# zeahmed/NeuralASR

Hardware: AMD Instinct MI355X
Metric: audio-frames/sec (fwd+bwd+CTC+Adam) at batch 16 per GPU (higher is better)
Workload: dtype f32

## Files before the change

neuralasr_amd/build.py:

```python
import os
import subprocess
import sys
from concurrent.futures import ThreadPoolExecutor

HERE = os.path.dirname(os.path.abspath(__file__))
CSRC = os.path.join(HERE, 'csrc')
LIB = os.path.join(HERE, 'libnasr.so')
KT_LIB = os.path.join(HERE, 'libnasr_kt.so')
KT_SRC = os.path.join(HERE, '..', 'tests', 'kernel_harness', 'harness.hip')
KT_OBJS = ['gemm.o', 'gemm_tph.o', 'optim.o']
SOURCES = ['gemm.hip', 'gemm_tph.hip', 'lstm.hip', 'lstm_persist.hip', 'lstm_wide.hip', 'ctc.hip', 'dense.hip', 'optim.hip', 'nasr_layout.hip',
           'nasr_rec.hip', 'nasr_batch.hip', 'nasr_pass.hip', 'nasr_api.hip', 'nasr_comm.hip', 'beam.cpp',
           'wavenet.hip', 'nasr_wavenet.hip', 'las.hip', 'las_beam.hip', 'nasr_las.hip', 'mfcc.hip', 'resample.hip']
HEADERS = [os.path.join(CSRC, 'kernels.h'), os.path.join(CSRC, 'lstm_device.h'), os.path.join(CSRC, 'nasr_ctx.h'), os.path.join(CSRC, 'wavenet.h'), os.path.join(CSRC, 'las.h'), os.path.join(CSRC, 'las_beam.h'), os.path.join(CSRC, 'resample.h'),
           os.path.join(HERE, '..', 'include', 'nasr.h')]
FLAGS = ['--offload-arch=gfx950', '-O3', '-std=c++17', '-fPIC', '-Wall', '-Wno-unused-function']


def _hipcc():
    for c in (os.environ.get('HIPCC'), '/opt/rocm/bin/hipcc', 'hipcc'):
        if c and (os.path.isabs(c) and os.path.exists(c) or not os.path.isabs(c)):
            return c
    return 'hipcc'


def _stale(target, deps):
    if not os.path.exists(target):
        return True
    t = os.path.getmtime(target)
    return any(os.path.getmtime(d) > t for d in deps if os.path.exists(d))


def build(force=False, verbose=False):
    hipcc = _hipcc()
    bdir = os.path.join(HERE, 'build')
    os.makedirs(bdir, exist_ok=True)
    jobs = []
    objs = []
    for s in SOURCES:
        src = os.path.join(CSRC, s)
        obj = os.path.join(bdir, os.path.splitext(s)[0] + '.o')
        objs.append(obj)
        if force or _stale(obj, [src] + HEADERS):
            jobs.append([hipcc] + FLAGS + ['-c', src, '-o', obj])

    def run(cmd):
        if verbose:
            print(' '.join(cmd), flush=True)
        r = subprocess.run(cmd, capture_output=True, text=True)
        if r.returncode != 0:
            raise RuntimeError('hipcc failed:\n' + ' '.join(cmd) + '\n' + r.stdout + r.stderr)
        if verbose and r.stderr.strip():
            print(r.stderr)

    kt_obj = os.path.join(bdir, 'kt_harness.o')
    if force or _stale(kt_obj, [KT_SRC] + HEADERS):
        jobs.append([hipcc] + FLAGS + ['-c', KT_SRC, '-o', kt_obj])

    with ThreadPoolExecutor(max_workers=min(4, max(1, len(jobs)))) as ex:
        list(ex.map(run, jobs))
    if force or jobs or _stale(LIB, objs):
        run([hipcc, '--offload-arch=gfx950', '-shared', '-fPIC', '-o', LIB] + objs + ['-lpthread'])
    kt_objs = [kt_obj] + [os.path.join(bdir, o) for o in KT_OBJS]
    if force or jobs or _stale(KT_LIB, kt_objs):
# ... 7 lines not shown
```

neuralasr_amd/csrc/kernels.h:

```cpp
#pragma once
#include <hip/hip_runtime.h>
#include <stdint.h>

namespace nasr {

const char* test_hook(const char* name);

struct GemmDesc {
  const float* A;
  const float* B;
  float* C;
  int M, N, K;
  int lda, ldb, ldc;
  bool a_col;
  bool b_col;
  const int* a_map;
  int a_shift;
  int a_rows;
  const int* c_map;
  const float* bias;
  int split_k;
  float* slabs;
};
void launch_gemm(const GemmDesc& g, hipStream_t st);
int gemm_pick_split(int M, int N, int K);

int tp_split2_parts(int rows);
int gemm_tp_tile_rows(int M);
size_t tph_bytes(int rows, int K);
size_t tph_scale_ws_floats(int rows, int K);
void launch_tph_scales(const float* src, int rows, int K, int ld, float* row_scale, float* row_inv, float* col_scale,
                       float* col_inv, float* ws, hipStream_t st);
constexpr int TPH_MAX_JOBS = 16;
struct TphScaleJob { const float* src; int rows, K, ld; float *row_scale, *row_inv, *col_scale, *col_inv; };
size_t tph_scale_batch_ws_floats(const TphScaleJob* jobs, int n);
void launch_tph_scales_batch(const TphScaleJob* jobs, int n, float* ws, hipStream_t st);
void launch_tph_scales_from_parts(const float* rowpart, int nrp, int rows, float* row_scale, float* row_inv, const float* colpart,
                                  int ncp, int K, float* col_scale, float* col_inv, hipStream_t st);
void launch_fill(float* p, float v, int n, hipStream_t st);
void launch_tph_split2(const float* src, unsigned char* tpN, unsigned char* tpT, int rows, int K, int ld,
                       const float* row_scale, float rs, const float* col_scale, float cs, float* colpart, hipStream_t st,
                       const int* rowmap = nullptr, const int* rowmap2 = nullptr, int col2 = 0);
void launch_gather_rows(float* dst, const float* src, const int* map, int n, float fill, hipStream_t st);
struct GemmTPHDesc {
  const unsigned char* A;
  const unsigned char* B;
  float* C;
  int M, N, K;
  int nkbA, nkbB;
  int ldc;
  int a_kshift;
  const float* bias;
  const float* a_inv;
  const float* b_inv;
  int split_k;
  float* slabs;
  int tile_rows;
  int nbatch;
  size_t a_bstride, b_bstride;
  int64_t c_bstride, ainv_bstride, binv_bstride;
  int a_kshift1;
  bool side;
  const int* c_map;
};
hipError_t gemm_tph_prepare();
int gemm_tph_pick_split(int M, int N, int K, int nbatch = 1);
void launch_gemm_tph(const GemmTPHDesc& g, hipStream_t st);

struct LstmDims {
  int T, B, Bp, H, Hp, D;
};
void launch_pack_feats(const float* feats_bm, float* X0, int B, int Bp, int T, int F, int Fp, hipStream_t st);
void launch_expand_context(const float* centre, const float* pad, const int* seq_len, float* X0, int B, int Bp, int T,
                           int ctx, int ncep, int Fp, hipStream_t st);
void launch_expand_context_masked(const float* centre, const float* pad, const int* seq_len, const int* masks, int nm,
                                  int static_width, float* X0, int B, int Bp, int T, int ctx, int ncep, int Fp,
                                  hipStream_t st);
void launch_repack_u(const float* U, float* Uf, float* Ub, int Hp, hipStream_t st);
// ... 102 lines not shown
```

neuralasr_amd/csrc/nasr_ctx.h:

```cpp
#pragma once
#include <hip/hip_runtime.h>

#include <dlfcn.h>
#include <sched.h>
#include <unistd.h>

#include <chrono>

#include <algorithm>
#include <cmath>
#include <cstdio>
#include <cstdlib>
#include <cstring>
#include <functional>
#include <map>
#include <memory>
#include <mutex>
#include <string>
#include <vector>

#include "../../include/nasr.h"
#include "kernels.h"
#include "resample.h"

// ... 117 lines not shown
  bool has_labels = false, centre = false;
  int64_t frames = 0;
  size_t o_seq = 0, o_lablen = 0, o_labels = 0, o_cstart = 0, o_cpos = 0, o_rowmap = 0;
  size_t o_vrow = 0, o_vprev = 0, o_vnext = 0;
  int Rv = 0, Rvp = 0;
  bool cmp = false;
  size_t nmeta = 0, nfeat = 0;
  size_t o_aug = 0;
  int aug_nm = 0, aug_sw = 0;
  bool masked = false;
  int32_t* meta_d() const { return dmeta.as<int32_t>(); }
};

enum class RecKind { Step = 0, Persist = 1, Wide = 2 };

enum class Family { Lstm, WaveNet, Las, Featurizer };

struct WnState;
struct WnStateDelete { void operator()(WnState* w) const; };
struct FzState;
struct FzStateDelete { void operator()(FzState* f) const; };
struct LasState;
struct LasStateDelete { void operator()(LasState* s) const; };

}

using namespace nasr;
using namespace nasr_impl;

struct nasr_ctx {

  nasr_model_cfg cfg;
  Family family = Family::Lstm;
  std::unique_ptr<WnState, WnStateDelete> wn;
  std::unique_ptr<FzState, FzStateDelete> fz;
  std::unique_ptr<LasState, LasStateDelete> las;
  int device = 0;
  Stream st;
  DevPtr<unsigned char> WfTP;
  DevPtr<unsigned char> WbTP;
  std::vector<size_t> off_wftp, off_wbtp;
  RecKind rec_kind = RecKind::Step;
  RecKind rec_use = RecKind::Step;
  bool rec_wanted = false;
  bool rec_inflight = false;
  bool rec_refused = false;
  int64_t rearm_after = 0, rearm_wait = 0, clean_steps = 0;
  int persist_aborts = 0, persist_rearms = 0;
  Pinned<unsigned> perr;
  DevPtr<float> Ucs, Ucinv;
  bool rec_f16 = false;
  DevPtr<float> Upf, Upb;
  size_t imf = 0, imb = 0;
  DevPtr<float> xchf;
  DevPtr<float> xchb;
  DevPtr<PersistCtl> pctl;
  DevPtr<unsigned char> Uw;
  DevPtr<unsigned char> Uwb;
  DevPtr<float> Urs, Urinv;
  DevPtr<float> wsrow;
  DevPtr<void> whx;
  DevPtr<float> wpart;
  DevPtr<void> wpx;
  DevPtr<WideCtl> wctl;
  void* comm = nullptr;
  void* comm2 = nullptr;
  Stream comm_st2;
  int comm_rank = 0, comm_n = 1;
  Stream comm_st;
  Event ev_comm;
  DevPtr<float> comm_scratch;

  int F, Fp, H, Hp, N4, D, L, C, Cp, Pin, Pinp;
  std::vector<int> Ip;
  std::vector<int64_t> off_wx, off_bias;
  std::vector<int64_t> off_u;
  int64_t off_w = 0, off_b = 0, np_int = 0;
  std::vector<TensorInfo> tensors;
  int64_t np_tf = 0;
  std::vector<int32_t> tf2int;

  int npre = 0, ndense = 0;
  bool has_post = false;
  int F0 = 0;
  std::vector<int> dWid, dWp, dIn, dIp;
  std::vector<int64_t> off_dw, off_db;
  std::vector<size_t> off_dftp, off_dbtp;
  DevPtr<unsigned char> DfTP, DbTP;
  std::vector<DevBuf> Ybuf, dYbuf;
  DevBuf DTP;
  uint32_t drop_seed = 4567u, drop_counter = 0;

  DevPtr<float> P, M, V, Uf, Ub;
  float* G = nullptr;
  struct SV {
    DevBuf s, inv;
    bool ensure(size_t n) { bool g = false; return s.ensure(n * 4, &g) && inv.ensure(n * 4, &g); }
    float* sp() const { return s.as<float>(); }
    float* ip() const { return inv.as<float>(); }
  };
  SV sc15;
  size_t sc15_n = 0;
  SV sc_x0r, sc_x0c;
  std::vector<SV> sc_yr, sc_yc;
  SV sc_gr, sc_gc;
  std::vector<SV> sc_wr, sc_wc;
  std::vector<SV> sc_dr, sc_dc;
  DevBuf scws;
  int gttp_layer = -1;
// ... 248 lines not shown
```

neuralasr_amd/csrc/nasr_pass.hip:

```cpp
#include "nasr_ctx.h"

using namespace nasr;
using namespace nasr_impl;

namespace nasr_impl {

int run_steps(nasr_ctx* h, int l, bool bwd, int s0, int s1, hipStream_t st, int* launches) {
  if (h->rec_use != RecKind::Step && s0 == 0 && s1 == h->T) return rec_launch(h, l, bwd, st, launches);
  *launches += s1 - s0;
  const LstmDims dm{h->T, h->B, h->Bp, h->H, h->Hp, h->D};
  const size_t sU = (size_t)l * h->D * h->Hp * h->N4;
  const size_t hs = (size_t)h->D * h->Bp * h->Hp;
  const size_t ps = (size_t)h->D * lstm_bwd_partials(h->Hp) * h->Bp * h->Hp;
  float* hst = h->hstate.as<float>();
  float* par = h->partial.as<float>();
  float* dcs = h->dcstate.as<float>();
  auto body = [&]() {
    if (!bwd) {
      if (s0 == 0) (void)hipMemsetAsync(hst, 0, hs * 4, st);
      for (int s = s0; s < s1; ++s)
        launch_lstm_fwd_step(dm, s, h->Uf + sU, hst + (s & 1) * hs, hst + ((s + 1) & 1) * hs,
                             h->gates[l].as<float>(), h->cbuf[l].as<float>(), h->outb[l].as<float>(),
                             h->seq_p, h->cfg.forget_bias, st);
    } else {
// ... 112 lines not shown
  pl_gemm(g, as.rinv, h->sc_dc[i].ip(), h->st);
  launch_dense_act(h->Ybuf[i].as<float>(), R, h->Bp, h->B, h->dWid[i], Wp, h->cfg.relu_clip, h->cfg.dropout[i],
                   h->drop_seed, h->drop_counter, i, h->st);
  pl_scales(h, h->Ybuf[i].as<float>(), R, Wp, Wp, &h->sc_yr[i], &h->sc_yc[i], h->st);
  HIPCHK(h, hipGetLastError());
  return NASR_OK;
}

int dense_backward(nasr_ctx* h, int i, const float* X, float* dX) {
  const int R = h->T * h->Bp, Ip = h->dIp[i], Wp = h->dWp[i];
  const int nkb = (R + 15) / 16;
  float* dZ = h->dYbuf[i].as<float>();
  launch_dense_act_bwd(dZ, h->Ybuf[i].as<float>(), (int64_t)R * Wp, h->cfg.relu_clip, h->cfg.dropout[i], h->st);
  const ActScale as = dense_in_scale(h, i);
  pl_scales(h, dZ, R, Wp, Wp, dX ? &h->sc_gr : nullptr, &h->sc_gc, h->st);
  pl_split(dZ, dX ? h->GTP.as<unsigned char>() : nullptr, h->GTTP.as<unsigned char>(), R, Wp, Wp, h->sc_gr.sp(),
           h->sc_gc.sp(), h->csws.as<float>(), h->st);
  pl_split(X, nullptr, h->DTP.as<unsigned char>(), R, Ip, Ip, nullptr, as.cs, nullptr, h->st);
  {
    GemmTPHDesc g{};
    g.A = h->DTP.as<unsigned char>(); g.B = h->GTTP.as<unsigned char>(); g.C = h->G + h->off_dw[i];
    g.M = Ip; g.N = Wp; g.K = R; g.nkbA = nkb; g.nkbB = nkb; g.ldc = Wp;
    g.split_k = gemm_tph_pick_split(g.M, g.N, g.K);
    g.slabs = ensure_slabs(h, g.split_k, g.M, g.N);
    if (g.split_k > 1 && !g.slabs) return h->fail(NASR_ERR_HIP, "slab workspace allocation failed");
    pl_gemm(g, as.cinv, h->sc_gc.ip(), h->st);
  }
  launch_colsum_parts(h->csws.as<float>(), tp_split2_parts(R), Wp, h->G + h->off_db[i], h->st);
  if (dX) {
    GemmTPHDesc g{};
    g.A = h->GTP.as<unsigned char>(); g.B = h->DbTP + h->off_dbtp[i]; g.C = dX;
    g.M = R; g.N = Ip; g.K = Wp; g.nkbA = (Wp + 15) / 16; g.nkbB = g.nkbA; g.ldc = Ip;
    g.split_k = gemm_tph_pick_split(g.M, g.N, g.K);
    g.slabs = ensure_slabs(h, g.split_k, g.M, g.N);
    if (g.split_k > 1 && !g.slabs) g.split_k = 1;
    pl_gemm(g, h->sc_gr.ip(), h->sc_dr[i].ip(), h->st);
  }
  HIPCHK(h, hipGetLastError());
  return NASR_OK;
}

int forward(nasr_ctx* h) {
  if (!h->resident) return h->fail(NASR_ERR_STATE, "no resident batch: call nasr_upload_batch first");
  switch (h->family) {
    case Family::WaveNet: return wn_forward(h, false);
    case Family::Las: return h->fail(NASR_ERR_STATE, "a LAS handle has no CTC logits: use nasr_las_forward");
    default: break;
  }
  const int Bp = h->Bp, T = h->T, D = h->D, Hp = h->Hp;
  const int R = T * Bp;
  h->n_fwd_launch = 0;
  std::fill(h->ott_valid.begin(), h->ott_valid.end(), 0);
  HIPCHK(h, hipMemsetAsync(h->Gbase, 0, GRAD_HEAD * 4, h->st));
  if (h->rec_use == RecKind::Persist) {
    HIPCHK(h, hipMemsetAsync(h->pctl + 1, 0, (size_t)h->L * sizeof(PersistCtl), h->st));
    HIPCHK(h, hipMemsetAsync(h->xchf, 0, (size_t)h->L * persist_hx_bytes(h->Hp), h->st));
  }
  for (int i = 0; i < h->npre; ++i) {
    PhaseScope ps(h, PH_XPROJ);
    int rc = dense_forward(h, i, i == 0 ? h->X0.as<float>() : h->Ybuf[i - 1].as<float>());
    if (rc) return rc;
  }
  for (int l = 0; l < h->L; ++l) {
    {
      PhaseScope ps(h, PH_XPROJ);
      gemm_xproj(h, l, R, h->st);
      HIPCHK(h, hipGetLastError());
    }
    PhaseScope ps(h, PH_RECF);
    int rc = run_steps(h, l, false, 0, T, h->st, &h->n_fwd_launch);
    if (rc) return rc;
  }
  if (h->has_post) {
    PhaseScope ps(h, PH_XPROJ);
    int rc = dense_forward(h, h->npre, h->outb[h->L - 1].as<float>());
    if (rc) return rc;
  }
  if (h->ndense) h->drop_counter += 1;
  {
    PhaseScope ps(h, PH_PROJCTC);
    const bool sr = h->cfg.merge == NASR_MERGE_STACK_RESHAPE && D == 2;
    GemmDesc g{};
    g.A = h->has_post ? h->Ybuf[h->npre].as<float>() : h->outb[h->L - 1].as<float>();
    g.B = h->P + h->off_w;
    g.C = h->logits.as<float>();
    g.M = h->Tp * Bp; g.N = h->Cp; g.K = h->Pinp;
    g.lda = sr ? Hp : h->Pinp; g.ldb = h->Cp; g.ldc = h->Cp;
    g.a_map = sr ? h->rowmap_p : nullptr;
    g.a_rows = sr ? 2 * R : R;
    g.bias = h->P + h->off_b;
    g.split_k = gemm_pick_split(g.M, g.N, g.K);
    if (int rc = gemm_f32(h, g)) return rc;
  }
  h->have_fwd = true;
  return NASR_OK;
}

CtcDims ctc_dims(nasr_ctx* h) {
  CtcDims d;
  d.Tp = h->Tp; d.B = h->B; d.Bp = h->Bp; d.C = h->C; d.Cp = h->Cp; d.Lmax = std::max(h->Lmax, 1);
  d.KS = h->KS; d.Tws = h->T + 8;
  d.lprobs = h->ctcprobs.as<float>(); d.goff = h->ctckexp.as<double>();
  return d;
}

int ctc_forward(nasr_ctx* h) {
  PhaseScope ps(h, PH_PROJCTC);
  const CtcDims d = ctc_dims(h);
  launch_ctc_logz(d, h->logits.as<float>(), h->seq_p, h->logz.as<float>(), h->st);
  launch_ctc_alpha_beta(d, h->logits.as<float>(), h->logz.as<float>(), h->labels_p, h->lablen_p,
                        h->seq_p, h->alpha.as<float>(), h->beta.as<float>(), h->aoff.as<double>(),
                        h->boff.as<double>(), h->nll.as<float>(), h->logp.as<double>(), h->st);
  launch_mean(h->nll.as<float>(), h->B, h->loss.as<float>(), h->st);
  if (h->step_decode) {
    if (h->step_greedy)
      launch_greedy(d, h->logits.as<float>(), h->seq_p, h->amax.as<int>(), h->ids.as<int>(), h->lens.as<int>(), h->st);
    h->have_decoded = h->step_greedy;
    h->res_cur ^= 1;
    nasr_ctx::StepRes& r = h->res[h->res_cur];
    const size_t ids_bytes = 8 + (size_t)h->Bp * 4 + (size_t)h->B * h->Tp * 4;
    const size_t lg_off = (ids_bytes + 255) / 256 * 256, lg_bytes = h->step_logits ? (size_t)h->Tp * h->Bp * h->Cp * 4 : 0;
    const size_t bytes = lg_off + lg_bytes;
    if (!pinned_ensure(r.host, &r.cap, bytes)) return h->fail(NASR_ERR_HIP, "hipHostMalloc of the step results failed");
    char* hp = static_cast<char*>(r.host.get());
    if (lg_bytes) {
      bool grew = false;
      if (!h->logits_snap.ensure(lg_bytes, &grew)) return h->fail(NASR_ERR_HIP, "hipMalloc of the logits snapshot failed");
      if (!r.ev_lg) HIPCHK(h, hipEventCreateWithFlags(r.ev_lg.out(), hipEventDisableTiming));
      nasr_ctx::StepRes& prev = h->res[h->res_cur ^ 1];
      if (prev.logits && prev.ev_lg) HIPCHK(h, hipStreamWaitEvent(h->st, prev.ev_lg, 0));
      HIPCHK(h, hipMemcpyAsync(h->logits_snap.p, h->logits.p, lg_bytes, hipMemcpyDeviceToDevice, h->st));
      HIPCHK(h, hipEventRecord(h->ev_snap, h->st));
      HIPCHK(h, hipStreamWaitEvent(h->d2h, h->ev_snap, 0));
      HIPCHK(h, hipMemcpyAsync(hp + lg_off, h->logits_snap.p, lg_bytes, hipMemcpyDeviceToHost, h->d2h));
      HIPCHK(h, hipEventRecord(r.ev_lg, h->d2h));
    }
    r.logits = lg_bytes != 0;
    r.seq = ++h->stamp_seq;
    launch_publish_results(h->loss.as<float>(), h->Gbase, h->lens.as<int>(), h->step_greedy ? h->Bp : 0, h->ids.as<int>(),
                           h->step_greedy ? h->B * h->Tp : 0, r.host, r.stamp, r.seq, h->st);
    r.greedy = h->step_greedy;
    r.valid = true; r.B = h->B; r.Bp = h->Bp; r.Tp = h->Tp;
  }
  HIPCHK(h, hipGetLastError());
  return NASR_OK;
// ... 41 lines not shown
  if (vm)
    launch_tph_split2(h->outb[l].as<float>(), nullptr, OS, rows, D * Hp, D * Hp, nullptr, 1.f, ao.cs, 1.f, nullptr, ws, h->vprev_p,
                      D == 2 ? h->vnext_p : nullptr, Hp);
  if (l == 0 && h->npre)
    pl_split(lstm_input(h, l), nullptr, h->X0TTP.as<unsigned char>(), R, h->Ip[0], h->Ip[0], nullptr, ai.cs, nullptr, ws);
  {
    GemmTPHDesc g{};
    g.A = l == 0 ? h->X0TTP.as<unsigned char>() : h->OTT[l - 1].as<unsigned char>();
    g.B = GT; g.C = h->G + h->off_wx[l];
    g.M = h->Ip[l]; g.N = D * N4; g.K = rows; g.nkbA = nkb; g.nkbB = nkb; g.ldc = D * N4;
    g.side = side;
    g.split_k = gemm_tph_pick_split(g.M, g.N, g.K);
    g.slabs = slabs_for(g.split_k, g.M, g.N);
    if (g.split_k > 1 && !g.slabs) return h->fail(NASR_ERR_HIP, "slab workspace allocation failed");
    pl_gemm(g, ai.cinv, gc.ip(), ws);
  }
  launch_colsum_parts(cs_part, tp_split2_parts(rows), D * N4, h->G + h->off_bias[l], ws);
  {
    GemmTPHDesc g{};
    g.A = vm ? OS : h->OTT[l].as<unsigned char>(); g.B = GT; g.C = h->G + h->off_u[(size_t)l * D];
    g.M = Hp; g.N = N4; g.K = rows; g.nkbA = nkb; g.nkbB = nkb; g.ldc = N4;
    g.a_kshift = vm ? 0 : -Bp;
    g.nbatch = D;
    g.a_bstride = (size_t)(Hp / 32) * pl_rb_bytes(nkb); g.b_bstride = (size_t)(N4 / 32) * pl_rb_bytes(nkb);
    g.c_bstride = (int64_t)Hp * N4;
    g.a_kshift1 = vm ? 0 : Bp;
    g.side = side;
    g.split_k = gemm_tph_pick_split(g.M, g.N, g.K, D);
    g.slabs = slabs_for(g.split_k * D, g.M, g.N);
    if (g.split_k > 1 && !g.slabs) return h->fail(NASR_ERR_HIP, "slab workspace allocation failed");
    pl_gemm(g, ao.cinv, gc.ip(), ws, Hp, N4);
  }
  HIPCHK(h, hipGetLastError());
  return NASR_OK;
}

int wg_join(nasr_ctx* h, int l) {
  if (l >= 0 && l < h->L && h->wg_pending[l]) {
    HIPCHK(h, hipStreamWaitEvent(h->st, h->ev_wg[l], 0));
    h->wg_pending[l] = 0;
  }
  return NASR_OK;
}

int backward(nasr_ctx* h) {
  switch (h->family) {
    case Family::WaveNet: return wn_backward(h);
    case Family::Las: return las_backward(h);
    default: break;
  }
  const int Bp = h->Bp, T = h->T, D = h->D, Hp = h->Hp;
  const int R = T * Bp, Rp = h->Tp * Bp;
  const bool sr = h->cfg.merge == NASR_MERGE_STACK_RESHAPE && D == 2;
  if (h->rec_use == RecKind::Persist) {
    HIPCHK(h, hipMemsetAsync(h->pctl + 1 + h->L, 0, (size_t)h->L * sizeof(PersistCtl), h->st));
    HIPCHK(h, hipMemsetAsync(h->xchb, 0, (size_t)h->L * persist_px_bytes(), h->st));
  }
  {
    PhaseScope ps(h, PH_PROJCTC);
    const CtcDims d = ctc_dims(h);
    launch_ctc_grad(d, h->logits.as<float>(), h->logz.as<float>(), h->lablen_p, h->seq_p,
                    h->cstart_p, h->cpos_p, h->alpha.as<float>(), h->beta.as<float>(),
                    h->aoff.as<double>(), h->boff.as<double>(), h->logp.as<double>(), 1.f / (float)h->B, h->st);
    HIPCHK(h, hipGetLastError());
  }
  {
    PhaseScope ps(h, PH_PROJB);
    GemmDesc g{};
    g.A = h->has_post ? h->Ybuf[h->npre].as<float>() : h->outb[h->L - 1].as<float>();
    g.B = h->logits.as<float>();
    g.C = h->G + h->off_w;
    g.M = h->Pinp; g.N = h->Cp; g.K = Rp;
    g.lda = sr ? Hp : h->Pinp; g.ldb = h->Cp; g.ldc = h->Cp;
    g.a_col = true; g.a_map = sr ? h->rowmap_p : nullptr; g.a_rows = sr ? 2 * R : R;
    g.split_k = gemm_pick_split(g.M, g.N, g.K);
    if (int rc = gemm_f32(h, g)) return rc;
    launch_colsum(h->logits.as<float>(), Rp, h->Cp, h->Cp, h->G + h->off_b, h->csws.as<float>(), h->st);
    GemmDesc x{};
    x.A = h->logits.as<float>();
    x.B = h->P + h->off_w;
    x.C = h->has_post ? h->dYbuf[h->npre].as<float>() : dout_of(h, h->L - 1);
    x.M = Rp; x.N = h->Pinp; x.K = h->Cp;
    x.lda = h->Cp; x.ldb = h->Cp; x.ldc = sr ? Hp : h->Pinp;
    x.b_col = true; x.a_rows = Rp; x.c_map = sr ? h->rowmap_p : nullptr; x.split_k = 1;
    if (int rc = gemm_f32(h, x)) return rc;
  }
  if (h->has_post) {
    PhaseScope ps(h, PH_WGRAD);
    int rc = dense_backward(h, h->npre, h->outb[h->L - 1].as<float>(), dout_of(h, h->L - 1));
    if (rc) return rc;
  }
  h->n_bwd_launch = 0;
  h->dgmax_layer = -1;
  for (int l = h->L - 1; l >= 0; --l) {
    const bool defer = h->rec_use != RecKind::Step && h->bucket_defer;
    {
      PhaseScope ps(h, PH_RECB);
      int rc = run_steps(h, l, true, 0, T, h->st, &h->n_bwd_launch);
      if (rc) return rc;
    }
    if (defer && l + 1 < h->L && h->bucket_of_layer[l + 1] >= 0) {
      if (int rc = wg_join(h, l + 1)) return rc;
      HIPCHK(h, hipEventRecord(h->ev_bucket[h->bucket_of_layer[l + 1]], h->st));
    }
    PhaseScope ps(h, PH_WGRAD);
    if (int rc = wg_join(h, l + 2)) return rc;
    if (l > 0 || h->npre > 0) gemm_dx(h, l, R, h->st);
    const bool side = h->wg_overlap && h->rec_use == RecKind::Persist && l > 0 && h->gttp_layer == l;
    if (side) {
      HIPCHK(h, hipEventRecord(h->ev_dx, h->st));
      HIPCHK(h, hipStreamWaitEvent(h->wst, h->ev_dx, 0));
      int rc = weight_grads(h, l, h->wst, true);
      if (rc) return rc;
      HIPCHK(h, hipEventRecord(h->ev_wg[l], h->wst));
      h->wg_pending[l] = 1;
    } else {
      int rc = weight_grads(h, l, h->st, false);
      if (rc) return rc;
    }
    if (h->bucket_of_layer[l] >= 0 && !(defer && l > 0)) {
      if (int rc = wg_join(h, l)) return rc;
      HIPCHK(h, hipEventRecord(h->ev_bucket[h->bucket_of_layer[l]], h->st));
    }
  }
  for (int l = 0; l < h->L; ++l)
    if (int rc = wg_join(h, l)) return rc;
  for (int i = h->npre - 1; i >= 0; --i) {
    PhaseScope ps(h, PH_WGRAD);
    int rc = dense_backward(h, i, i == 0 ? h->X0.as<float>() : h->Ybuf[i - 1].as<float>(),
                            i > 0 ? h->dYbuf[i - 1].as<float>() : nullptr);
// ... 21 lines not shown
```

neuralasr_amd/csrc/nasr_rec.hip:

```cpp
#include "nasr_ctx.h"

namespace nasr_impl {

static bool persist_census(nasr_ctx* h) {
  const int Bp = 16, T = 2;
  const size_t R = (size_t)T * Bp;
  DevBuf g, c, o, dg, sq;
  bool grew = false;
  bool ok = g.ensure(R * h->D * h->N4 * 4, &grew) && c.ensure(R * h->D * h->Hp * 4, &grew) &&
            o.ensure(R * h->D * h->Hp * 4, &grew) && dg.ensure(R * h->D * h->N4 * 4, &grew) && sq.ensure(Bp * 4, &grew);
  if (ok) {
    (void)hipMemsetAsync(g.p, 0, R * h->D * h->N4 * 4, h->st);
    (void)hipMemsetAsync(o.p, 0, R * h->D * h->Hp * 4, h->st);
    std::vector<int32_t> two((size_t)Bp, T);
    (void)hipMemcpyAsync(sq.p, two.data(), Bp * 4, hipMemcpyHostToDevice, h->st);
    const LstmDims dm{T, Bp, Bp, h->H, h->Hp, h->D};
    launch_lstm_persist_fwd(dm, h->Upf, h->rec_f16 ? h->Ucinv : nullptr, g.as<float>(), c.as<float>(), o.as<float>(),
                            sq.as<int>(), h->xchf, h->pctl, h->perr, nullptr, 1.f, h->st);
    launch_lstm_persist_bwd(dm, h->Upb, g.as<float>(), dg.as<float>(), c.as<float>(), o.as<float>(), sq.as<int>(),
                            h->xchb, h->pctl, h->perr, nullptr, h->st, false, nullptr, nullptr, h->bwd_lean);
    ok = hipStreamSynchronize(h->st) == hipSuccess && hipGetLastError() == hipSuccess && *h->perr == 0;
  }
  *h->perr = 0;
  return ok;
}

int rec_setup(nasr_ctx* h, bool allowed, bool f32) {
  h->rec_kind = !allowed ? RecKind::Step : persist_supported(h->Hp) ? RecKind::Persist
                : wide_supported(h->Hp, 16) ? RecKind::Wide : RecKind::Step;
  if (h->rec_kind == RecKind::Step) return NASR_OK;
  h->rec_f16 = h->rec_kind == RecKind::Persist && !f32;
  const size_t nk = (size_t)h->L * h->D;
  bool g2 = false;
  if (hipHostMalloc(h->perr.out(), 64, hipHostMallocMapped) != hipSuccess || hipMalloc(h->Ucs.out(), nk * h->N4 * 4) != hipSuccess ||
      hipMalloc(h->Ucinv.out(), nk * h->N4 * 4) != hipSuccess || !h->scws.ensure(nk * tph_scale_ws_floats(h->Hp, h->N4) * 4, &g2))
    return h->fail(NASR_ERR_HIP, "allocation of the recurrent-weight scales failed");
  *h->perr = 0;
  if (h->rec_f16) {
    (void)hipMemsetAsync(h->Ucs, 0, nk * h->N4 * 4, h->st);
    (void)hipMemsetAsync(h->Ucinv, 0, nk * h->N4 * 4, h->st);
  }
  if (h->rec_kind == RecKind::Persist) {
    h->imf = persist_image_floats(h->Hp, false);
    h->imb = persist_image_floats(h->Hp, true);
    if (persist_prepare() != hipSuccess || hipMalloc(h->Upf.out(), nk * h->imf * 4) != hipSuccess ||
        hipMalloc(h->Upb.out(), nk * h->imb * 4) != hipSuccess ||
        hipMalloc(h->xchf.out(), (size_t)h->L * persist_hx_bytes(h->Hp)) != hipSuccess ||
        hipMalloc(h->xchb.out(), (size_t)h->L * persist_px_bytes()) != hipSuccess ||
        hipMalloc(h->pctl.out(), (size_t)(1 + 2 * h->L) * sizeof(PersistCtl)) != hipSuccess)
      return h->fail(NASR_ERR_HIP, "allocation of the persistent-recurrence buffers failed");
    (void)hipMemsetAsync(h->Upf, 0, nk * h->imf * 4, h->st);
    (void)hipMemsetAsync(h->Upb, 0, nk * h->imb * 4, h->st);
    return NASR_OK;
  }
  if (wide_prepare() != hipSuccess || hipMalloc(h->Uw.out(), nk * wide_image_bytes(h->Hp)) != hipSuccess ||
      hipMalloc(h->whx.out(), wide_hx_bytes(64)) != hipSuccess || hipMalloc(h->wpart.out(), wide_part_bytes(64)) != hipSuccess ||
      hipMalloc(h->wctl.out(), sizeof(WideCtl)) != hipSuccess || hipMalloc(h->Uwb.out(), nk * wide_image_bytes(h->Hp)) != hipSuccess ||
      hipMalloc(h->wpx.out(), wide_px_bytes(64)) != hipSuccess || hipMalloc(h->Urs.out(), nk * h->Hp * 4) != hipSuccess ||
      hipMalloc(h->Urinv.out(), nk * h->Hp * 4) != hipSuccess || hipMalloc(h->wsrow.out(), 2 * 64 * 4) != hipSuccess)
    return h->fail(NASR_ERR_HIP, "allocation of the wide persistent-recurrence buffers failed");
  (void)hipMemsetAsync(h->whx, 0, wide_hx_bytes(64), h->st);
  (void)hipMemsetAsync(h->wpx, 0, wide_px_bytes(64), h->st);
  return NASR_OK;
}

void rec_start(nasr_ctx* h) {
  if (h->rec_kind == RecKind::Persist && !persist_census(h)) h->rec_kind = RecKind::Step;
  h->rec_use = h->rec_kind;
  h->rec_wanted = h->rec_kind != RecKind::Step;
}

int rec_launch(nasr_ctx* h, int l, bool bwd, hipStream_t st, int* launches) {
  const LstmDims dm{h->T, h->B, h->Bp, h->H, h->Hp, h->D};
  if (h->rec_use == RecKind::Persist) {
    const size_t k = (size_t)l * h->D;
    if (!bwd) {
      launch_lstm_persist_fwd(dm, h->Upf + k * h->imf, h->rec_f16 ? h->Ucinv + k * h->N4 : nullptr,
                              h->gates[l].as<float>(), h->cbuf[l].as<float>(),
                              h->outb[l].as<float>(), h->seq_p, h->xchf + (size_t)l * (persist_hx_bytes(h->Hp) / 4),
                              h->pctl + 1 + l, h->perr, h->Gbase, h->cfg.forget_bias, st, true);
    } else {
      launch_lstm_persist_bwd(dm, h->Upb + k * h->imb, h->gates[l].as<float>(), dg_of(h, l), h->cbuf[l].as<float>(),
                              dout_of(h, l), h->seq_p, h->xchb + (size_t)l * (persist_px_bytes() / 4), h->pctl + 1 + h->L + l,
                              h->perr, h->Gbase, st, true, h->dgmax.as<float>(),
                              h->dgmax.as<float>() + (size_t)h->D * 32 * h->T * h->Bp, h->bwd_lean);
      h->dgmax_layer = l;
    }
    *launches += 1;
  } else {
    if (bwd) launch_wide_row_scales(dm, dout_of(h, l), h->seq_p, h->wsrow, st);
    for (int d = 0; d < h->D; ++d) {
      const size_t k = (size_t)l * h->D + d;
      if (!bwd)
        launch_lstm_wide_fwd(dm, d, h->Uw + k * wide_image_bytes(h->Hp), h->Ucinv + k * h->N4, h->gates[l].as<float>(),
                             h->cbuf[l].as<float>(), h->outb[l].as<float>(), h->seq_p, h->whx, h->wpart, h->wctl, h->perr,
                             h->Gbase, h->cfg.forget_bias, st);
      else
        launch_lstm_wide_bwd(dm, d, h->Uwb + k * wide_image_bytes(h->Hp), h->Urinv + k * h->Hp, h->wsrow,
                             h->gates[l].as<float>(), dg_of(h, l), h->cbuf[l].as<float>(), dout_of(h, l), h->seq_p, h->wpart,
                             h->wpx, h->wctl, h->perr, h->Gbase, st);
    }
    *launches += h->D;
  }
  h->rec_inflight = true;
  HIPCHK(h, hipGetLastError());
  return NASR_OK;
}

int rec_check(nasr_ctx* h) {
  if (!h->rec_inflight) return NASR_OK;
  h->rec_inflight = false;
  const unsigned code = *reinterpret_cast<volatile unsigned*>(h->perr.get());
  if (!code) return NASR_OK;
  *reinterpret_cast<volatile unsigned*>(h->perr.get()) = 0;
  h->rec_use = RecKind::Step;
  h->rec_refused = true;
  h->persist_aborts += 1;
  h->clean_steps = 0;
  h->rearm_wait = h->persist_aborts <= 1 ? h->rearm_after : std::min<int64_t>(h->rearm_wait * 2, (int64_t)1 << 20);
  (void)repack(h);
  return h->fail(NASR_ERR_HIP, "persistent recurrence aborted (code " + std::to_string(code) +
                                   ": 1 = hand-off timeout, 2 = workgroup placement, 4 = dG beyond its fp16 planes); the results of this step are "
                                   "invalid, later steps use the per-step kernels" +
                                   (h->rearm_wait > 0 ? " (the persistent kernels are tried again after " +
                                                            std::to_string(h->rearm_wait) + " clean steps)"
                                                      : ""));
}

void rec_rearm(nasr_ctx* h) {
  if (h->rec_use != RecKind::Step || !h->rec_wanted || h->persist_aborts == 0 || h->rearm_wait <= 0) return;
  if (++h->clean_steps <= h->rearm_wait) return;
  h->clean_steps = 0;
  if (hipStreamSynchronize(h->st) != hipSuccess) return;
  h->rec_use = h->rec_kind;
  if (repack(h) != NASR_OK || (h->rec_kind == RecKind::Persist && !persist_census(h))) {
    h->rec_use = RecKind::Step;
// ... 57 lines not shown
```

Before: 1.201 million.

## Add specialized MFMA kernels for narrow output projection and merge persist memsets

```diff
diff --git a/neuralasr_amd/build.py b/neuralasr_amd/build.py
--- a/neuralasr_amd/build.py
+++ b/neuralasr_amd/build.py
@@ -9,7 +9,7 @@
 KT_LIB = os.path.join(HERE, 'libnasr_kt.so')
 KT_SRC = os.path.join(HERE, '..', 'tests', 'kernel_harness', 'harness.hip')
 KT_OBJS = ['gemm.o', 'gemm_tph.o', 'optim.o']
-SOURCES = ['gemm.hip', 'gemm_tph.hip', 'lstm.hip', 'lstm_persist.hip', 'lstm_wide.hip', 'ctc.hip', 'dense.hip', 'optim.hip', 'nasr_layout.hip',
+SOURCES = ['gemm.hip', 'gemm_tph.hip', 'proj.hip', 'lstm.hip', 'lstm_persist.hip', 'lstm_wide.hip', 'ctc.hip', 'dense.hip', 'optim.hip', 'nasr_layout.hip',
            'nasr_rec.hip', 'nasr_batch.hip', 'nasr_pass.hip', 'nasr_api.hip', 'nasr_comm.hip', 'beam.cpp',
            'wavenet.hip', 'nasr_wavenet.hip', 'las.hip', 'las_beam.hip', 'nasr_las.hip', 'mfcc.hip', 'resample.hip']
 HEADERS = [os.path.join(CSRC, 'kernels.h'), os.path.join(CSRC, 'lstm_device.h'), os.path.join(CSRC, 'nasr_ctx.h'), os.path.join(CSRC, 'wavenet.h'), os.path.join(CSRC, 'las.h'), os.path.join(CSRC, 'las_beam.h'), os.path.join(CSRC, 'resample.h'),
diff --git a/neuralasr_amd/csrc/kernels.h b/neuralasr_amd/csrc/kernels.h
--- a/neuralasr_amd/csrc/kernels.h
+++ b/neuralasr_amd/csrc/kernels.h
@@ -24,6 +24,14 @@
 };
 void launch_gemm(const GemmDesc& g, hipStream_t st);
 int gemm_pick_split(int M, int N, int K);
+
+bool proj_supported(int Cp, int K, int lda, int a_rows, int Rp);
+void launch_proj_fwd(const float* A, const int* a_map, int a_rows, int lda, const float* W, const float* bias, float* logits,
+                     int Rp, int K, hipStream_t st);
+int proj_wgrad_slices(int Rp);
+size_t proj_wgrad_slab_floats(int Rp, int K);
+void launch_proj_wgrad(const float* A, const int* a_map, int a_rows, int lda, const float* dlogits, int Rp, int K, float* dW,
+                       float* db, float* slabs, hipStream_t st);
 
 int tp_split2_parts(int rows);
 int gemm_tp_tile_rows(int M);
diff --git a/neuralasr_amd/csrc/nasr_ctx.h b/neuralasr_amd/csrc/nasr_ctx.h
--- a/neuralasr_amd/csrc/nasr_ctx.h
+++ b/neuralasr_amd/csrc/nasr_ctx.h
@@ -193,9 +193,13 @@
   bool rec_f16 = false;
   DevPtr<float> Upf, Upb;
   size_t imf = 0, imb = 0;
-  DevPtr<float> xchf;
-  DevPtr<float> xchb;
-  DevPtr<PersistCtl> pctl;
+  DevPtr<unsigned char> pmem;
+  float* xchb = nullptr;
+  PersistCtl* pctlb = nullptr;
+  float* xchf = nullptr;
+  PersistCtl* pctlf = nullptr;
+  PersistCtl* pctl = nullptr;
+  size_t pclr_f = 0, pclr_b = 0;
   DevPtr<unsigned char> Uw;
   DevPtr<unsigned char> Uwb;
   DevPtr<float> Urs, Urinv;
diff --git a/neuralasr_amd/csrc/nasr_pass.hip b/neuralasr_amd/csrc/nasr_pass.hip
--- a/neuralasr_amd/csrc/nasr_pass.hip
+++ b/neuralasr_amd/csrc/nasr_pass.hip
@@ -188,10 +188,7 @@
   h->n_fwd_launch = 0;
   std::fill(h->ott_valid.begin(), h->ott_valid.end(), 0);
   HIPCHK(h, hipMemsetAsync(h->Gbase, 0, GRAD_HEAD * 4, h->st));
-  if (h->rec_use == RecKind::Persist) {
-    HIPCHK(h, hipMemsetAsync(h->pctl + 1, 0, (size_t)h->L * sizeof(PersistCtl), h->st));
-    HIPCHK(h, hipMemsetAsync(h->xchf, 0, (size_t)h->L * persist_hx_bytes(h->Hp), h->st));
-  }
+  if (h->rec_use == RecKind::Persist) HIPCHK(h, hipMemsetAsync(h->xchf, 0, h->pclr_f, h->st));
   for (int i = 0; i < h->npre; ++i) {
     PhaseScope ps(h, PH_XPROJ);
     int rc = dense_forward(h, i, i == 0 ? h->X0.as<float>() : h->Ybuf[i - 1].as<float>());
@@ -225,8 +222,13 @@
     g.a_map = sr ? h->rowmap_p : nullptr;
     g.a_rows = sr ? 2 * R : R;
     g.bias = h->P + h->off_b;
-    g.split_k = gemm_pick_split(g.M, g.N, g.K);
-    if (int rc = gemm_f32(h, g)) return rc;
+    if (proj_supported(h->Cp, g.K, g.lda, g.a_rows, g.M)) {
+      launch_proj_fwd(g.A, g.a_map, g.a_rows, g.lda, g.B, g.bias, g.C, g.M, g.K, h->st);
+      HIPCHK(h, hipGetLastError());
+    } else {
+      g.split_k = gemm_pick_split(g.M, g.N, g.K);
+      if (int rc = gemm_f32(h, g)) return rc;
+    }
   }
   h->have_fwd = true;
   return NASR_OK;
@@ -374,10 +376,7 @@
   const int Bp = h->Bp, T = h->T, D = h->D, Hp = h->Hp;
   const int R = T * Bp, Rp = h->Tp * Bp;
   const bool sr = h->cfg.merge == NASR_MERGE_STACK_RESHAPE && D == 2;
-  if (h->rec_use == RecKind::Persist) {
-    HIPCHK(h, hipMemsetAsync(h->pctl + 1 + h->L, 0, (size_t)h->L * sizeof(PersistCtl), h->st));
-    HIPCHK(h, hipMemsetAsync(h->xchb, 0, (size_t)h->L * persist_px_bytes(), h->st));
-  }
+  if (h->rec_use == RecKind::Persist) HIPCHK(h, hipMemsetAsync(h->xchb, 0, h->pclr_b, h->st));
   {
     PhaseScope ps(h, PH_PROJCTC);
     const CtcDims d = ctc_dims(h);
@@ -395,9 +394,16 @@
     g.M = h->Pinp; g.N = h->Cp; g.K = Rp;
     g.lda = sr ? Hp : h->Pinp; g.ldb = h->Cp; g.ldc = h->Cp;
     g.a_col = true; g.a_map = sr ? h->rowmap_p : nullptr; g.a_rows = sr ? 2 * R : R;
-    g.split_k = gemm_pick_split(g.M, g.N, g.K);
-    if (int rc = gemm_f32(h, g)) return rc;
-    launch_colsum(h->logits.as<float>(), Rp, h->Cp, h->Cp, h->G + h->off_b, h->csws.as<float>(), h->st);
+    if (proj_supported(h->Cp, g.M, g.lda, g.a_rows, Rp)) {
+      bool grew = false;
+      if (!h->slabs.ensure(proj_wgrad_slab_floats(Rp, g.M) * 4, &grew)) return h->fail(NASR_ERR_HIP, "slab workspace allocation failed");
+      launch_proj_wgrad(g.A, g.a_map, g.a_rows, g.lda, g.B, Rp, g.M, g.C, h->G + h->off_b, h->slabs.as<float>(), h->st);
+      HIPCHK(h, hipGetLastError());
+    } else {
+      g.split_k = gemm_pick_split(g.M, g.N, g.K);
+      if (int rc = gemm_f32(h, g)) return rc;
+      launch_colsum(h->logits.as<float>(), Rp, h->Cp, h->Cp, h->G + h->off_b, h->csws.as<float>(), h->st);
+    }
     GemmDesc x{};
     x.A = h->logits.as<float>();
     x.B = h->P + h->off_w;
diff --git a/neuralasr_amd/csrc/nasr_rec.hip b/neuralasr_amd/csrc/nasr_rec.hip
--- a/neuralasr_amd/csrc/nasr_rec.hip
+++ b/neuralasr_amd/csrc/nasr_rec.hip
@@ -43,12 +43,20 @@
   if (h->rec_kind == RecKind::Persist) {
     h->imf = persist_image_floats(h->Hp, false);
     h->imb = persist_image_floats(h->Hp, true);
+    const size_t ctlb = (size_t)h->L * sizeof(PersistCtl), al = (size_t)2 << 20;
+    h->pclr_b = (size_t)h->L * persist_px_bytes() + ctlb;
+    h->pclr_f = (size_t)h->L * persist_hx_bytes(h->Hp) + ctlb;
+    const size_t off_f = (h->pclr_b + al - 1) / al * al;
     if (persist_prepare() != hipSuccess || hipMalloc(h->Upf.out(), nk * h->imf * 4) != hipSuccess ||
         hipMalloc(h->Upb.out(), nk * h->imb * 4) != hipSuccess ||
-        hipMalloc(h->xchf.out(), (size_t)h->L * persist_hx_bytes(h->Hp)) != hipSuccess ||
-        hipMalloc(h->xchb.out(), (size_t)h->L * persist_px_bytes()) != hipSuccess ||
-        hipMalloc(h->pctl.out(), (size_t)(1 + 2 * h->L) * sizeof(PersistCtl)) != hipSuccess)
+        hipMalloc(h->pmem.out(), off_f + h->pclr_f + sizeof(PersistCtl)) != hipSuccess)
       return h->fail(NASR_ERR_HIP, "allocation of the persistent-recurrence buffers failed");
+    unsigned char* pm = h->pmem;
+    h->xchb = reinterpret_cast<float*>(pm);
+    h->pctlb = reinterpret_cast<PersistCtl*>(pm + h->pclr_b - ctlb);
+    h->xchf = reinterpret_cast<float*>(pm + off_f);
+    h->pctlf = reinterpret_cast<PersistCtl*>(pm + off_f + h->pclr_f - ctlb);
+    h->pctl = h->pctlf + h->L;
     (void)hipMemsetAsync(h->Upf, 0, nk * h->imf * 4, h->st);
     (void)hipMemsetAsync(h->Upb, 0, nk * h->imb * 4, h->st);
     return NASR_OK;
@@ -78,10 +86,10 @@
       launch_lstm_persist_fwd(dm, h->Upf + k * h->imf, h->rec_f16 ? h->Ucinv + k * h->N4 : nullptr,
                               h->gates[l].as<float>(), h->cbuf[l].as<float>(),
                               h->outb[l].as<float>(), h->seq_p, h->xchf + (size_t)l * (persist_hx_bytes(h->Hp) / 4),
-                              h->pctl + 1 + l, h->perr, h->Gbase, h->cfg.forget_bias, st, true);
+                              h->pctlf + l, h->perr, h->Gbase, h->cfg.forget_bias, st, true);
     } else {
       launch_lstm_persist_bwd(dm, h->Upb + k * h->imb, h->gates[l].as<float>(), dg_of(h, l), h->cbuf[l].as<float>(),
-                              dout_of(h, l), h->seq_p, h->xchb + (size_t)l * (persist_px_bytes() / 4), h->pctl + 1 + h->L + l,
+                              dout_of(h, l), h->seq_p, h->xchb + (size_t)l * (persist_px_bytes() / 4), h->pctlb + l,
                               h->perr, h->Gbase, st, true, h->dgmax.as<float>(),
                               h->dgmax.as<float>() + (size_t)h->D * 32 * h->T * h->Bp, h->bwd_lean);
       h->dgmax_layer = l;
diff --git a/neuralasr_amd/csrc/proj.hip b/neuralasr_amd/csrc/proj.hip
--- /dev/null
+++ b/neuralasr_amd/csrc/proj.hip
@@ -0,0 +1,237 @@
+#include "kernels.h"
+
+namespace nasr {
+
+typedef float f32x16 __attribute__((ext_vector_type(16)));
+
+namespace {
+
+constexpr int PC = 32;
+constexpr int PF_ROWS = 32;
+constexpr int PF_KU = 64;
+constexpr int PW_KB = 128;
+constexpr int PW_ROWS = 128;
+constexpr int PW_MAXS = 64;
+constexpr int PW_RU = 32;
+
+struct ProjParams {
+  const float* A;
+  const float* W;
+  const float* bias;
+  float* C;
+  const int* a_map;
+  int Rp, K, lda, a_rows;
+  int rows_per;
+};
+
+template <bool MAP>
+__device__ __forceinline__ int proj_row(const int* __restrict__ map, int rows, int logical) {
+  const int r = MAP ? map[logical] : logical;
+  return (r >= 0 && r < rows) ? r : -1;
+}
+
+template <bool MAP>
+__global__ __launch_bounds__(256) void proj_fwd_kernel(ProjParams p) {
+  __shared__ float red[4][PF_ROWS][PC + 1];
+  const int tid = threadIdx.x, lane = tid & 63, w = tid >> 6;
+  const int li = lane & 31, hh = lane >> 5;
+  const int m = blockIdx.x * PF_ROWS + li;
+  const int prm = proj_row<MAP>(p.a_map, p.a_rows, min(m, p.Rp - 1));
+  const int pr = m < p.Rp ? prm : -1;
+  const float* __restrict__ arow = p.A + (pr >= 0 ? (size_t)pr * p.lda : 0);
+  const float* __restrict__ W = p.W;
+  const int kq = ((p.K + 3) / 4 + PF_KU - 1) / PF_KU * PF_KU;
+  const int kbeg = w * kq, kend = min(p.K, kbeg + kq);
+
+  f32x16 acc;
+#pragma unroll
+  for (int r = 0; r < 16; ++r) acc[r] = 0.f;
+
+  float4 a[PF_KU / 8], an[PF_KU / 8];
+  float b[PF_KU / 2], bn[PF_KU / 2];
+  auto load = [&](int k0, float4* av, float* bv) {
+#pragma unroll
+    for (int u = 0; u < PF_KU / 8; ++u) {
+      const int k = k0 + 8 * u + 4 * hh;
+      const bool ok = k < kend;
+      const float4 v = *reinterpret_cast<const float4*>(arow + (ok ? k : 0));
+      const bool ua = ok && pr >= 0;
+      av[u] = make_float4(ua ? v.x : 0.f, ua ? v.y : 0.f, ua ? v.z : 0.f, ua ? v.w : 0.f);
+#pragma unroll
+      for (int j = 0; j < 4; ++j) {
+        const float wv = W[(size_t)(ok ? k + j : 0) * PC + li];
+        bv[4 * u + j] = ok ? wv : 0.f;
+      }
+    }
+  };
+  load(kbeg, a, b);
+  for (int k0 = kbeg; k0 < kend; k0 += PF_KU) {
+    load(k0 + PF_KU, an, bn);
+#pragma unroll
+    for (int u = 0; u < PF_KU / 8; ++u) {
+      acc = __builtin_amdgcn_mfma_f32_32x32x2f32(a[u].x, b[4 * u + 0], acc, 0, 0, 0);
+      acc = __builtin_amdgcn_mfma_f32_32x32x2f32(a[u].y, b[4 * u + 1], acc, 0, 0, 0);
+      acc = __builtin_amdgcn_mfma_f32_32x32x2f32(a[u].z, b[4 * u + 2], acc, 0, 0, 0);
+      acc = __builtin_amdgcn_mfma_f32_32x32x2f32(a[u].w, b[4 * u + 3], acc, 0, 0, 0);
+    }
+#pragma unroll
+    for (int u = 0; u < PF_KU / 8; ++u) a[u] = an[u];
+#pragma unroll
+    for (int u = 0; u < PF_KU / 2; ++u) b[u] = bn[u];
+  }
+#pragma unroll
+  for (int r = 0; r < 16; ++r) red[w][(r & 3) + 8 * (r >> 2) + 4 * hh][li] = acc[r];
+  __syncthreads();
+#pragma unroll
+  for (int e = 0; e < PF_ROWS * PC / 256; ++e) {
+    const int idx = tid + 256 * e, row = idx >> 5, col = idx & 31;
+    const int mo = blockIdx.x * PF_ROWS + row;
+    if (mo < p.Rp) {
+      const float s = ((red[0][row][col] + red[1][row][col]) + red[2][row][col]) + red[3][row][col];
+      p.C[(size_t)mo * PC + col] = s + p.bias[col];
+    }
+  }
+}
+
+template <bool MAP>
+__global__ __launch_bounds__(256) void proj_wgrad_kernel(ProjParams p) {
+  const int tid = threadIdx.x, lane = tid & 63, w = tid >> 6;
+  const int li = lane & 31, hh = lane >> 5;
+  const int kc = blockIdx.x * PW_KB + w * 32;
+  const bool kok = kc + li < p.K;
+  const int rbeg = blockIdx.y * p.rows_per, rend = min(p.Rp, rbeg + p.rows_per);
+  const __amdgpu_buffer_rsrc_t Ab = __builtin_amdgcn_make_buffer_rsrc(const_cast<float*>(p.A), 0, p.a_rows * p.lda * 4, 0x00020000);
+  const __amdgpu_buffer_rsrc_t Db = __builtin_amdgcn_make_buffer_rsrc(const_cast<float*>(p.W), 0, p.Rp * PC * 4, 0x00020000);
+  constexpr int OOB = -4;
+
+  f32x16 acc;
+#pragma unroll
+  for (int r = 0; r < 16; ++r) acc[r] = 0.f;
+  float dbs = 0.f;
+
+  float a[PW_RU / 2], an[PW_RU / 2], b[PW_RU / 2], bn[PW_RU / 2];
+  int pr[PW_RU / 2];
+  auto rows = [&](int r0) {
+#pragma unroll
+    for (int u = 0; u < PW_RU / 2; ++u) {
+      const int r = r0 + 2 * u + hh;
+      pr[u] = proj_row<MAP>(p.a_map, p.a_rows, r < rend ? r : rbeg);
+    }
+  };
+  auto load = [&](int r0, float* av, float* bv) {
+#pragma unroll
+    for (int u = 0; u < PW_RU / 2; ++u) {
+      const int r = r0 + 2 * u + hh;
+      const bool rok = r < rend;
+      if constexpr (MAP) asm volatile("" : "+v"(pr[u]));
+      const int ao = (rok && pr[u] >= 0 && kok) ? (pr[u] * p.lda + kc + li) * 4 : OOB;
+      av[u] = __builtin_bit_cast(float, __builtin_amdgcn_raw_buffer_load_b32(Ab, ao, 0, 0));
+      bv[u] = __builtin_bit_cast(float, __builtin_amdgcn_raw_buffer_load_b32(Db, rok ? (r * PC + li) * 4 : OOB, 0, 0));
+    }
+  };
+  rows(rbeg);
+  load(rbeg, a, b);
+  rows(rbeg + PW_RU);
+  for (int r0 = rbeg; r0 < rend; r0 += PW_RU) {
+    load(r0 + PW_RU, an, bn);
+    rows(r0 + 2 * PW_RU);
+#pragma unroll
+    for (int u = 0; u < PW_RU / 2; ++u) {
+      acc = __builtin_amdgcn_mfma_f32_32x32x2f32(a[u], b[u], acc, 0, 0, 0);
+      dbs += b[u];
+    }
+#pragma unroll
+    for (int u = 0; u < PW_RU / 2; ++u) { a[u] = an[u]; b[u] = bn[u]; }
+  }
+  float* slab = p.C + (size_t)blockIdx.y * (p.K + 1) * PC;
+#pragma unroll
+  for (int r = 0; r < 16; ++r) {
+    const int k = kc + (r & 3) + 8 * (r >> 2) + 4 * hh;
+    if (k < p.K) slab[(size_t)k * PC + li] = acc[r];
+  }
+  if (blockIdx.x == 0 && w == 0) {
+    const float other = __shfl_xor(dbs, 32);
+    if (hh == 0) slab[(size_t)p.K * PC + li] = dbs + other;
+  }
+}
+
+__global__ __launch_bounds__(256) void proj_wgrad_reduce_kernel(const float* __restrict__ slabs, int S, int K, float* dW,
+                                                                float* db) {
+  __shared__ float4 part[8][32];
+  const int o = threadIdx.x & 31, g = threadIdx.x >> 5;
+  const int n4 = (K + 1) * PC / 4;
+  const int i = blockIdx.x * 32 + o;
+  const int per = (S + 7) / 8;
+  float4 v[PW_MAXS / 8];
+#pragma unroll
+  for (int j = 0; j < PW_MAXS / 8; ++j) {
+    const int sl = g * per + j;
+    const bool ok = j < per && sl < S && i < n4;
+    const float4 x = *reinterpret_cast<const float4*>(slabs + (ok ? ((size_t)sl * n4 + i) * 4 : 0));
+    v[j] = make_float4(ok ? x.x : 0.f, ok ? x.y : 0.f, ok ? x.z : 0.f, ok ? x.w : 0.f);
+  }
+  float4 s = v[0];
+#pragma unroll
+  for (int j = 1; j < PW_MAXS / 8; ++j) { s.x += v[j].x; s.y += v[j].y; s.z += v[j].z; s.w += v[j].w; }
+  part[g][o] = s;
+  __syncthreads();
+  if (g != 0 || i >= n4) return;
+#pragma unroll
+  for (int k = 1; k < 8; ++k) {
+    const float4 x = part[k][o];
+    s.x += x.x; s.y += x.y; s.z += x.z; s.w += x.w;
+  }
+  const int row = i / (PC / 4), c4 = i % (PC / 4);
+  if (row < K) {
+    *reinterpret_cast<float4*>(dW + (size_t)row * PC + 4 * c4) = s;
+  } else {
+    float* d = db + 4 * c4;
+    d[0] = s.x; d[1] = s.y; d[2] = s.z; d[3] = s.w;
+  }
+}
+
+int wgrad_rows_per(int Rp) {
+  int per = PW_ROWS;
+  while ((Rp + per - 1) / per > PW_MAXS) per *= 2;
+  return per;
+}
+
+}
+
+bool proj_supported(int Cp, int K, int lda, int a_rows, int Rp) {
+  return Cp == PC && K > 0 && K % 4 == 0 && lda % 4 == 0 && (size_t)a_rows * lda * 4 < ((size_t)1 << 31) &&
+         (size_t)Rp * PC * 4 < ((size_t)1 << 31);
+}
+
+void launch_proj_fwd(const float* A, const int* a_map, int a_rows, int lda, const float* W, const float* bias, float* logits,
+                     int Rp, int K, hipStream_t st) {
+  ProjParams p{};
+  p.A = A; p.W = W; p.bias = bias; p.C = logits; p.a_map = a_map;
+  p.Rp = Rp; p.K = K; p.lda = lda; p.a_rows = a_rows;
+  const dim3 grid((Rp + PF_ROWS - 1) / PF_ROWS), block(256);
+  if (a_map) hipLaunchKernelGGL(proj_fwd_kernel<true>, grid, block, 0, st, p);
+  else hipLaunchKernelGGL(proj_fwd_kernel<false>, grid, block, 0, st, p);
+}
+
+int proj_wgrad_slices(int Rp) {
+  const int per = wgrad_rows_per(Rp);
+  return (Rp + per - 1) / per;
+}
+
+size_t proj_wgrad_slab_floats(int Rp, int K) { return (size_t)proj_wgrad_slices(Rp) * (K + 1) * PC; }
+
+void launch_proj_wgrad(const float* A, const int* a_map, int a_rows, int lda, const float* dlogits, int Rp, int K, float* dW,
+                       float* db, float* slabs, hipStream_t st) {
+  ProjParams p{};
+  p.A = A; p.W = dlogits; p.C = slabs; p.a_map = a_map;
+  p.Rp = Rp; p.K = K; p.lda = lda; p.a_rows = a_rows;
+  p.rows_per = wgrad_rows_per(Rp);
+  const int S = proj_wgrad_slices(Rp);
+  const dim3 grid((K + PW_KB - 1) / PW_KB, S), block(256);
+  if (a_map) hipLaunchKernelGGL(proj_wgrad_kernel<true>, grid, block, 0, st, p);
+  else hipLaunchKernelGGL(proj_wgrad_kernel<false>, grid, block, 0, st, p);
+  const int n4 = (K + 1) * PC / 4;
+  hipLaunchKernelGGL(proj_wgrad_reduce_kernel, dim3((n4 + 31) / 32), dim3(256), 0, st, slabs, S, K, dW, db);
+}
+
+}
```

New measurement: 1.211 million, median of 6. No clear change (+0.9%).
